# LordLiang/DrawingSpinUp

Hardware: AMD Instinct MI355X
Metric: drawings/sec end-to-end (512x512, 6 views, 24 frames) (higher is better)
Workload: dtype f16 (diffusion) / f16 table + f32 MLP (NSR) / f32 (stage-1 deformable convolutions, IS-Net, contour) / f32 with bf16 x 3 products (stage-2 convolutions; the reference: cuDNN TF32)

## Files before the change

drawingspinup_amd/csrc/hashgrid_mfma.hip:

```cpp
#include "hashgrid_dev.h"
#include "partial_reduce.h"

#include <type_traits>

using namespace dsu_hg;

namespace {

typedef float f32x16 __attribute__((ext_vector_type(16)));
typedef __bf16 bf16x8 __attribute__((ext_vector_type(8)));

__device__ __forceinline__ void softplus_inplace2(f32x16& acc, int r) {
  const f32x2 h = softplus100_pair(f32x2{acc[r], acc[r + 1]});
  acc[r] = h.x;
  acc[r + 1] = h.y;
}

__device__ __forceinline__ void bf16_split8(const float* x, bf16x8& hi, bf16x8& mid) {
#pragma unroll
  for (int i = 0; i < 8; ++i) {
    const __bf16 h = (__bf16)x[i];
    hi[i] = h;
    mid[i] = (__bf16)(x[i] - (float)h);
  }
// ... 922 lines not shown
      for (int l = 0; l < ACT; ++l) vm_take(rw[l]);
      prep_unpack();
      prep_point(e);
      prep_request(e);
      prep_dout(e);
    }
#pragma unroll 1
    for (; e < 7; e += e_step) {
      gb1[0] += dout0;
      const float other0 = partner32(dout0, h);
      const float d0h0 = h == 0 ? dout0 : other0;
      const float d0h1 = h == 1 ? dout0 : other0;
      bf16x8 obh0, obm0, obh1, obm1;
      if constexpr (L0BF)
        pack_operands(in, std::integral_constant<int, (2 * KPA <= 16 ? 2 * KPA : 16)>{}, obh0, obm0, obh1, obm1);
#pragma unroll
      for (int half = 0; half < 2; ++half) {
        if (half == 1 && !live1) break;
        weights_per_use();
        const float d0 = half ? d0h1 : d0h0;
        f32x16 Hh[2];
        if constexpr (L0BF) l0_bf(half ? obh1 : obh0, half ? obm1 : obm0, Hh);
        else l0_half(in, half, Hh);
        softplus2(Hh);
#pragma unroll
        for (int T = 0; T < 2; ++T)
#pragma unroll
          for (int r = 0; r < 16; ++r) gw1c0[T][r] = fmaf(Hh[T][r], d0, gw1c0[T][r]);
        f32x16 din;
#pragma unroll
        for (int r = 0; r < 16; ++r) din[r] = 0.0f;
#pragma unroll
        for (int T = 0; T < 2; ++T) {
          float dpre[16];
#pragma unroll
          for (int q = 0; q < 4; ++q) {
            const float4 w = *reinterpret_cast<const float4*>(&lds[wo + PW_W1O0 + 32 * T + 8 * q + 4 * h]);
            dpre[4 * q + 0] = w.x * d0;
            dpre[4 * q + 1] = w.y * d0;
            dpre[4 * q + 2] = w.z * d0;
            dpre[4 * q + 3] = w.w * d0;
          }
          din_tile(T, dpre, Hh[T], din);
        }
        if (h == half) stage_in_T(in);
        __builtin_amdgcn_wave_barrier();
        gemm_T(gw0, imgI);
        __builtin_amdgcn_wave_barrier();
        store_din(e, din, wave_first + half * 32 + l31, r1);
      }
      const int en = e + e_step < 7 ? e + e_step : 6;
      handover();
      prep_unpack();
      prep_point(en);
      prep_request(en);
      prep_dout(en);
    }
#pragma unroll
    for (int T = 0; T < 2; ++T)
#pragma unroll
      for (int r = 0; r < 16; ++r) {
        float c0 = gw1c0[T][r];
#pragma unroll
        for (int off = 16; off > 0; off >>= 1) c0 += __shfl_xor(c0, off);
        if (l31 == gw1_col(0)) gw0[T][r] += c0;
      }
  }

  __syncthreads();
  float* red = lds;
  {
    float* rr = red + wave * PART_STRIDE;
#pragma unroll
    for (int T = 0; T < 2; ++T)
#pragma unroll
      for (int r = 0; r < 16; ++r) {
        const int feat = feat_of(T, r, h);
        const bool input = l31 < 2 * ACT || (l31 >= 2 * NL && l31 < 2 * NL + 4);
        rr[PART_GW0 + feat * 32 + l31] = input ? gw0[T][r] : 0.0f;
        const int o = l31 >= 2 * NL + 4 ? l31 - (2 * NL + 4) : (l31 >= 2 * ACT && l31 < 2 * ACT + NOUT - 8 ? l31 - 2 * ACT + 8 : -1);
        if (o >= 0) rr[PART_GW1 + feat * 32 + o] = gw0[T][r];
        if (l31 >= NOUT) rr[PART_GW1 + feat * 32 + l31] = 0.0f;
      }
#pragma unroll
    for (int o = 0; o < NOUT; ++o) gb1[o] += __shfl_xor(gb1[o], 32);
#pragma unroll
    for (int off = 16; off > 0; off >>= 1)
#pragma unroll
      for (int o = 0; o < NOUT; ++o) gb1[o] += __shfl_xor(gb1[o], off);
    if (lane == 0) {
#pragma unroll
      for (int o = 0; o < NOUT; ++o) rr[PART_GB1 + o] = gb1[o];
    }
  }
  __syncthreads();
  float* part = partials + (size_t)blockIdx.x * PART_STRIDE;
  for (int v = threadIdx.x; v < PART_GB1 + NOUT; v += blockDim.x)
    part[v] = (red[v] + red[PART_STRIDE + v]) + (red[2 * PART_STRIDE + v] + red[3 * PART_STRIDE + v]);
}

template <int NL, int ACT>
bool launch_bwd_pipe_one(uint32_t active, int blocks, hipStream_t s, const dsu_sdf_mlp& mlp,
                         const float* pts, int64_t n, float radius, float eps, float eps2,
                         const float* d_sdf, const float* d_grad, const float* d_feature,
                         const float* d_laplace, float* partials, const __half2* enc, float2* dinbuf,
                         const int32_t* perm) {
  if ((int)active != ACT) return false;
  sdf_fd_bwd_pipe_kernel<NL, ACT><<<dim3(blocks), dim3(256), 0, s>>>(
      mlp, pts, n, radius, eps, eps2, d_sdf, d_grad, d_feature, d_laplace, partials, enc, dinbuf, perm);
  return true;
}

template <int NL>
bool launch_bwd_pipe(uint32_t active, int blocks, hipStream_t s, const dsu_sdf_mlp& mlp,
                     const float* pts, int64_t n, float radius, float eps, float eps2,
                     const float* d_sdf, const float* d_grad, const float* d_feature,
                     const float* d_laplace, float* partials, const __half2* enc, float2* dinbuf,
                     const int32_t* perm) {
#define DSU_PIPE_TRY(A)                                                                          \
  if (launch_bwd_pipe_one<NL, A>(active, blocks, s, mlp, pts, n, radius, eps, eps2, d_sdf,       \
                                 d_grad, d_feature, d_laplace, partials, enc, dinbuf, perm))      \
    return true;
  DSU_PIPE_TRY(4) DSU_PIPE_TRY(5) DSU_PIPE_TRY(6) DSU_PIPE_TRY(7)
#undef DSU_PIPE_TRY
  return false;
}

constexpr int SC_MAXBLOCKS = 768;
constexpr int SC_THREADS = 256;
constexpr int SC_QCAP = 512;
constexpr int SC_LOG2 = 10;
constexpr int SC_SLOTS = 1 << SC_LOG2;
constexpr int SC_LDS_F = SC_SLOTS + 4 * SC_SLOTS + (SC_THREADS / 64) * 3 * SC_QCAP;
constexpr int SC_TILE_CAP = (SC_LDS_F * 4) / 16;
constexpr int SC_BBOX_OFF = SC_LDS_F;
constexpr int SC_LDS_TOTAL = SC_LDS_F + 16;
static_assert(SC_QCAP % 4 == 0 && SC_QCAP >= 512, "queue: one full evaluation of a wave must fit");

__device__ __forceinline__ uint32_t sc_slot(uint32_t entry) {
  return (entry * 2654435761u) >> (32 - SC_LOG2);
}
__device__ __forceinline__ void sc_commit_from(uint32_t* keys, unsigned long long* acc,
                                               float* __restrict__ gtable, uint32_t entry,
                                               uint32_t slot, float v0, float v1) {
#pragma unroll
  for (int probe = 1; probe < 3; ++probe) {
    slot = (slot + 1) & (SC_SLOTS - 1);
    const uint32_t old = atomicCAS(&keys[slot], GC_EMPTY, entry);
    if (old == GC_EMPTY || old == entry) {
      atomicAdd(&acc[2 * slot], gc_fix(v0));
      atomicAdd(&acc[2 * slot + 1], gc_fix(v1));
      return;
    }
  }
  unsafeAtomicAdd(gtable + (size_t)entry * 2, v0);
  unsafeAtomicAdd(gtable + (size_t)entry * 2 + 1, v1);
}

struct OwnReduce {
  const float* partials;
  int nblocks;
  float *g_w0, *g_b0, *g_w1, *g_b1;
};
constexpr int OWN_RED_BLOCKS = (PART_GB1 + NOUT + 63) / 64;

template <int NL>
__device__ __forceinline__ void reduce_own_block(const OwnReduce& o, int blk, float* red) {
  const int e = threadIdx.x & 63, g = threadIdx.x >> 6, ng = blockDim.x >> 6;
  const int v = blk * 64 + e;
  const bool in_range = v < PART_GB1 + NOUT;
  for (int sl = g; sl < 16; sl += ng) {
    float acc = 0.0f;
    if (in_range)
      for (int b = sl; b < o.nblocks; b += 16) acc += o.partials[(size_t)b * PART_STRIDE + v];
    red[sl * 64 + e] = acc;
  }
  __syncthreads();
  if (g != 0 || !in_range) return;
  float s = 0.0f;
#pragma unroll
  for (int k = 0; k < 16; ++k) s += red[k * 64 + e];
  if (v < PART_GW1) {
    const int feat = v >> 5, k = v & 31;
    if (k < MC<NL>::KIN) {
      const int c = ref_col<NL>(k);
      if (c >= 0) o.g_w0[feat * MC<NL>::DIN + c] += s;
      else o.g_b0[feat] += s;
    }
  } else if (v < PART_GB1) {
    const int feat = (v - PART_GW1) >> 5, oo = (v - PART_GW1) & 31;
    if (oo < NOUT) o.g_w1[oo * HID + feat] += s;
  } else {
    o.g_b1[v - PART_GB1] += s;
  }
}

template <int NL>
__global__ __launch_bounds__(SC_THREADS) void sdf_fd_scatter_kernel(
    GridMeta m, const float* __restrict__ pts, int64_t n, float radius, float eps, uint32_t active,
    const float2* __restrict__ dinbuf, float* __restrict__ gtable, int merge_levels,
    int centre_acc, int dense_levels, int* __restrict__ work_counter, OwnReduce own,
    dsu_partial_reduce extra) {
  extern __shared__ __attribute__((aligned(16))) float lds[];
  const int n_red_own = own.partials ? OWN_RED_BLOCKS : 0;
  const int n_red = n_red_own + (extra.partials ? dsu_red::blocks_of(extra) : 0);
  if ((int)blockIdx.x < n_red) {
    if ((int)blockIdx.x < n_red_own) reduce_own_block<NL>(own, blockIdx.x, lds);
    else dsu_red::reduce_block(extra, blockIdx.x - n_red_own, lds);
    return;
  }
  const int sc_block = (int)blockIdx.x - n_red, sc_grid = (int)gridDim.x - n_red;
  uint32_t* c_keys = reinterpret_cast<uint32_t*>(lds);
  unsigned long long* c_acc = reinterpret_cast<unsigned long long*>(lds + SC_SLOTS);
  const int lane = threadIdx.x & 63, wave = threadIdx.x >> 6;
  float* qbase = lds + 5 * SC_SLOTS + wave * 3 * SC_QCAP;
  uint32_t* q_ent = reinterpret_cast<uint32_t*>(qbase);
  float* q_v0 = qbase + SC_QCAP;
  float* q_v1 = qbase + 2 * SC_QCAP;
  unsigned long long* tile = reinterpret_cast<unsigned long long*>(lds);
  int* bbox = reinterpret_cast<int*>(lds + SC_BBOX_OFF);
  for (int t = threadIdx.x; t < SC_SLOTS; t += blockDim.x) {
    c_keys[t] = GC_EMPTY;
    c_acc[2 * t] = 0ull;
    c_acc[2 * t + 1] = 0ull;
  }
  if (threadIdx.x < 12) bbox[threadIdx.x] = (threadIdx.x % 6) < 3 ? 0x7fffffff : -0x7fffffff;
  int region = 0;
  __syncthreads();
  const int64_t n_chunks = (n + blockDim.x - 1) / blockDim.x;
  const int64_t n_items = n_chunks * (int64_t)active;
  int* next_slot = reinterpret_cast<int*>(lds + SC_BBOX_OFF) + 12;
  int64_t cur = sc_block, nxt = (int64_t)sc_block + sc_grid;
  float pn[3] = {0.f, 0.f, 0.f};
  float2 dnx[7];
#pragma unroll
  for (int e = 0; e < 7; ++e) dnx[e] = make_float2(0.f, 0.f);
  auto request = [&](int64_t item) {
    const int64_t chunk = item / (int64_t)active;
    const uint32_t lv = (uint32_t)(item - chunk * (int64_t)active);
    int64_t idx = chunk * blockDim.x + threadIdx.x;
    idx = idx < n ? idx : n - 1;
    pn[0] = pts[idx * 3]; pn[1] = pts[idx * 3 + 1]; pn[2] = pts[idx * 3 + 2];
#pragma unroll
    for (int e = 0; e < 7; ++e) dnx[e] = dinbuf[((size_t)e * active + lv) * n + idx];
  };
  if (cur < n_items) request(cur);
  int parity = 0;
  int qn = 0;
  auto drain = [&]() {
    __builtin_amdgcn_wave_barrier();
    for (int i0 = 0; i0 < qn; i0 += 64) {
      const int qi = i0 + lane;
      if (qi < qn) {
        const uint32_t ent = q_ent[qi];
        const float a0 = q_v0[qi], a1 = q_v1[qi];
        const uint32_t slot = sc_slot(ent);
        const uint32_t old = atomicCAS(&c_keys[slot], GC_EMPTY, ent);
        if (old == GC_EMPTY || old == ent) {
          atomicAdd(&c_acc[2 * slot], gc_fix(a0));
          atomicAdd(&c_acc[2 * slot + 1], gc_fix(a1));
        } else {
          sc_commit_from(c_keys, c_acc, gtable, ent, slot, a0, a1);
        }
      }
    }
    __builtin_amdgcn_wave_barrier();
    qn = 0;
  };
  auto flush_cache = [&]() {
    for (int t = threadIdx.x; t < SC_SLOTS; t += blockDim.x) {
      const uint32_t key = c_keys[t];
      if (key != GC_EMPTY) {
        unsafeAtomicAdd(gtable + (size_t)key * 2, gc_unfix(c_acc[2 * t]));
        unsafeAtomicAdd(gtable + (size_t)key * 2 + 1, gc_unfix(c_acc[2 * t + 1]));
        c_keys[t] = GC_EMPTY;
        c_acc[2 * t] = 0ull;
        c_acc[2 * t + 1] = 0ull;
      }
    }
  };

#pragma unroll 1
  while (cur < n_items) {
    {
      const int64_t chunk = cur / (int64_t)active;
      const int lev = (int)(cur - chunk * (int64_t)active);
      const float l_scale = m.scale[lev];
      const uint32_t l_off = m.off[lev], hsize = m.off[lev + 1] - m.off[lev];
      const uint32_t l_res = m.res[lev], l_hashed = m.hashed[lev];
      const int64_t i = chunk * blockDim.x + threadIdx.x;
      const bool valid = i < n;
      const float p[3] = {pn[0], pn[1], pn[2]};
      float2 dv[7];
#pragma unroll
      for (int e = 0; e < 7; ++e) {
        dv[e].x = valid ? dnx[e].x : 0.0f;
        dv[e].y = valid ? dnx[e].y : 0.0f;
      }
      if (nxt < n_items) request(nxt);
      if (threadIdx.x == 0) *next_slot = 2 * sc_grid + atomicAdd(work_counter, 1);
      const CellPos ccp = cell_of(l_scale, contract(p[0], radius), contract(p[1], radius),
                                  contract(p[2], radius));
      float2 D0 = dv[0], Da[3];
      uint32_t left = 0u;
      const bool inside = fabsf(p[0]) <= radius && fabsf(p[1]) <= radius && fabsf(p[2]) <= radius;
      int lo[3], hi[3];
#pragma unroll
      for (int a = 0; a < 3; ++a) {
        Da[a] = make_float2(0.f, 0.f);
        lo[a] = valid ? (int)ccp.c[a] : 0x7fffffff;
        hi[a] = valid ? (int)ccp.c[a] : -0x7fffffff;
      }
#pragma unroll
      for (int e = 1; e < 7; ++e) {
        const int ax = (e - 1) >> 1;
        const float off = ((e - 1) & 1) ? -eps : eps;
        const float qa = fminf(fmaxf(p[ax] + off, -radius), radius);
        const float posa = fmaf(l_scale, contract(qa, radius), 0.5f);
        const float fl = floorf(posa);
        const bool same = ((uint32_t)(int)fl == ccp.c[ax]) & (centre_acc != 0) & inside;
        const float delta = posa - ((float)(int)ccp.c[ax] + ccp.f[ax]);
        D0.x += same ? dv[e].x : 0.0f;
        D0.y += same ? dv[e].y : 0.0f;
        Da[ax].x += same ? dv[e].x * delta : 0.0f;
        Da[ax].y += same ? dv[e].y * delta : 0.0f;
        left |= (valid & !same) ? (1u << e) : 0u;
        if (valid & inside) {
          lo[ax] = min(lo[ax], (int)fl);
          hi[ax] = max(hi[ax], (int)fl);
        }
      }
      if (valid & !inside) {
#pragma unroll 1
        for (int e = 1; e < 7; ++e) {
          float q[3];
          fd_point(p, e, eps, radius, q);
          const CellPos cq = cell_of(l_scale, contract(q[0], radius), contract(q[1], radius),
                                     contract(q[2], radius));
#pragma unroll
          for (int a = 0; a < 3; ++a) {
            lo[a] = min(lo[a], (int)cq.c[a]);
            hi[a] = max(hi[a], (int)cq.c[a]);
          }
        }
      }
      bool dense = false;
      int x0 = 0, y0 = 0, z0 = 0, ddx = 1, ddxy = 1, vol = 0;
      int64_t after_next;
      {
        int* bb = bbox + 6 * parity;
#pragma unroll
        for (int a = 0; a < 3; ++a) {
#pragma unroll
          for (int off = 32; off > 0; off >>= 1) {
            lo[a] = min(lo[a], __shfl_xor(lo[a], off));
            hi[a] = max(hi[a], __shfl_xor(hi[a], off));
          }
        }
        if (lane == 0) {
#pragma unroll
          for (int a = 0; a < 3; ++a) {
            atomicMin(&bb[a], lo[a]);
            atomicMax(&bb[3 + a], hi[a]);
          }
        }
        __syncthreads();
        after_next = *next_slot;
        x0 = bb[0]; y0 = bb[1]; z0 = bb[2];
        const long long ex = (long long)bb[3] - x0 + 2, ey = (long long)bb[4] - y0 + 2,
                        ez = (long long)bb[5] - z0 + 2;
        if (dense_levels && bb[3] >= bb[0] && ex * ey * ez <= (long long)SC_TILE_CAP && ex < 4096 && ey < 4096) {
          dense = true;
          ddx = (int)ex; ddxy = (int)(ex * ey); vol = (int)(ex * ey * ez);
        }
        if (threadIdx.x < 6) bbox[6 * (parity ^ 1) + threadIdx.x] = threadIdx.x < 3 ? 0x7fffffff : -0x7fffffff;
        parity ^= 1;
      }
      if ((int)dense != region) {
        if (region == 0) {
          for (int t = threadIdx.x; t < SC_TILE_CAP * 2; t += blockDim.x) tile[t] = 0ull;
        } else {
          for (int t = threadIdx.x; t < SC_SLOTS; t += blockDim.x) {
            c_keys[t] = GC_EMPTY;
            c_acc[2 * t] = 0ull;
            c_acc[2 * t + 1] = 0ull;
          }
        }
        region = (int)dense;
        __syncthreads();
      }

#pragma unroll 1
      for (int e = 1; e < 8; ++e) {
        CellPos cp = ccp;
        float v[16];
        bool flush;
        if (e < 7) {
          flush = (left >> e) & 1u;
          if (__ballot(flush) == 0ull) continue;
          float2 d = dv[1];
#pragma unroll
          for (int k = 2; k < 7; ++k) {
            d.x = e == k ? dv[k].x : d.x;
            d.y = e == k ? dv[k].y : d.y;
          }
          float q[3];
          fd_point(p, e, eps, radius, q);
          cp = cell_of(l_scale, contract(q[0], radius), contract(q[1], radius), contract(q[2], radius));
#pragma unroll
          for (int c = 0; c < 8; ++c) {
            const float w = corner_weight(cp, c);
            v[2 * c] = w * d.x;
            v[2 * c + 1] = w * d.y;
          }
        } else {
          const float X[2] = {1.0f - cp.f[0], cp.f[0]}, Y[2] = {1.0f - cp.f[1], cp.f[1]},
                      Z[2] = {1.0f - cp.f[2], cp.f[2]};
#pragma unroll
          for (int c = 0; c < 8; ++c) {
            const int cx_ = c & 1, cy_ = (c >> 1) & 1, cz_ = (c >> 2) & 1;
            const float yz = Y[cy_] * Z[cz_], xz = X[cx_] * Z[cz_], xy = X[cx_] * Y[cy_];
            const float w = X[cx_] * yz;
            const float gx = cx_ ? yz : -yz, gy = cy_ ? xz : -xz, gz = cz_ ? xy : -xy;
            v[2 * c] = fmaf(D0.x, w, fmaf(Da[0].x, gx, fmaf(Da[1].x, gy, Da[2].x * gz)));
            v[2 * c + 1] = fmaf(D0.y, w, fmaf(Da[0].y, gx, fmaf(Da[1].y, gy, Da[2].y * gz)));
          }
          flush = valid;
        }
        const int key = flush ? (int)((cp.c[0] & 1023u) | ((cp.c[1] & 1023u) << 10) | ((cp.c[2] & 1023u) << 20))
                              : (0x40000000 | lane);
#pragma unroll
        for (int k = 0; k < 16; ++k) v[k] = flush ? v[k] : 0.0f;
        bool lead = flush;
        const int key_next = dpp_i<0x101>(key), key_prev = dpp_i<0x111>(key);
        const int l15 = lane & 15;
        const bool starts = ((l15 == 0) | (key_prev != key)) & flush;
        const int n_flush = __popcll(__ballot(flush)), n_start = __popcll(__ballot(starts));
        if (lev < merge_levels && 4 * n_start <= 3 * n_flush) {
          int ee = ((l15 == 15) | (key_next != key)) ? 1 : 0;
#define DSU_SEG_STEP(CTRL)                                              \
          {                                                             \
            const int eo = dpp_i<CTRL>(ee);                             \
            _Pragma("unroll") for (int k = 0; k < 16; ++k) {            \
              const float vo = dpp_f<CTRL>(v[k]);                       \
              v[k] += ee ? 0.0f : vo;                                   \
            }                                                           \
            ee |= eo;                                                   \
          }
          DSU_SEG_STEP(0x101) DSU_SEG_STEP(0x102) DSU_SEG_STEP(0x104) DSU_SEG_STEP(0x108)
#undef DSU_SEG_STEP
          lead = starts;
        }
        if (dense) {
          if (lead) {
            const int base = ((int)cp.c[0] - x0) + ((int)cp.c[1] - y0) * ddx + ((int)cp.c[2] - z0) * ddxy;
#pragma unroll
            for (int c = 0; c < 8; ++c) {
              const int t = base + (c & 1) + ((c >> 1) & 1) * ddx + ((c >> 2) & 1) * ddxy;
              atomicAdd(&tile[2 * t], gc_fix(v[2 * c]));
              atomicAdd(&tile[2 * t + 1], gc_fix(v[2 * c + 1]));
            }
          }
          continue;
        }
        const unsigned long long bal = __ballot(lead);
        if (lead) {
          const int pos = qn + 8 * __popcll(bal & ((1ull << lane) - 1ull));
          uint32_t ent[8];
#pragma unroll
          for (int c = 0; c < 8; ++c)
            ent[c] = l_off + grid_index(l_hashed, hsize, l_res, cp.c[0] + (c & 1),
                                        cp.c[1] + ((c >> 1) & 1), cp.c[2] + ((c >> 2) & 1));
#pragma unroll
          for (int q4 = 0; q4 < 2; ++q4) {
            *reinterpret_cast<uint4*>(&q_ent[pos + 4 * q4]) =
                make_uint4(ent[4 * q4], ent[4 * q4 + 1], ent[4 * q4 + 2], ent[4 * q4 + 3]);
            *reinterpret_cast<float4*>(&q_v0[pos + 4 * q4]) =
                make_float4(v[8 * q4], v[8 * q4 + 2], v[8 * q4 + 4], v[8 * q4 + 6]);
            *reinterpret_cast<float4*>(&q_v1[pos + 4 * q4]) =
                make_float4(v[8 * q4 + 1], v[8 * q4 + 3], v[8 * q4 + 5], v[8 * q4 + 7]);
          }
        }
        qn += 8 * __popcll(bal);
        if (qn + 512 > SC_QCAP) drain();
      }
      if (!dense) drain();
      __syncthreads();
      if (dense) {
        for (int t = threadIdx.x; t < vol; t += blockDim.x) {
          const unsigned long long a0 = tile[2 * t], a1 = tile[2 * t + 1];
          if (a0 | a1) {
            const int z = t / ddxy, rr = t - z * ddxy;
            const int y = rr / ddx, x = rr - y * ddx;
            const uint32_t g = l_off + grid_index(l_hashed, hsize, l_res, (uint32_t)(x0 + x),
                                                  (uint32_t)(y0 + y), (uint32_t)(z0 + z));
            unsafeAtomicAdd(gtable + (size_t)g * 2, gc_unfix(a0));
            unsafeAtomicAdd(gtable + (size_t)g * 2 + 1, gc_unfix(a1));
            tile[2 * t] = 0ull;
            tile[2 * t + 1] = 0ull;
          }
        }
      } else {
        flush_cache();
      }
      cur = nxt;
      nxt = after_next;
    }
  }
}

constexpr int BWD_MFMA_MAX_BLOCKS = 512;

}

#define DSU_DISPATCH_NL(nl, ...)                       \
  switch (nl) {                                        \
    case 10: { constexpr int NL = 10; __VA_ARGS__ } break; \
    case 12: { constexpr int NL = 12; __VA_ARGS__ } break; \
    default: return DSU_EUNSUP;                        \
  }

extern "C" {

int64_t dsu_sdf_fd_enc_cache_bytes(int64_t n, uint32_t active_levels) {
  if (n < 0 || active_levels > DSU_MAX_LEVELS) return DSU_EINVAL;
  return (int64_t)7 * n * active_levels * 4;
}

int64_t dsu_sdf_fd_bwd_workspace_bytes(const dsu_hashgrid_cfg* cfg, int64_t n) {
  if (!cfg || n < 0) return DSU_EINVAL;
  if (cfg->n_levels != 10 && cfg->n_levels != 12) return DSU_EUNSUP;
  const int blocks = dsu_capped_blocks(n, 256, BWD_MFMA_MAX_BLOCKS);
  return (int64_t)blocks * PART_STRIDE * sizeof(float) +
         (int64_t)7 * n * cfg->n_levels * (int64_t)sizeof(float2) + 256;
}

int dsu_sdf_fd_bwd_sorted(const dsu_hashgrid_cfg* cfg, const void* table_f16, const dsu_sdf_mlp* mlp,
                   const float* pts, const int32_t* perm, int64_t n, float radius, float eps,
                   uint32_t active_levels, const float* d_sdf, const float* d_grad,
                   const float* d_feature, const float* d_laplace, float* grad_table,
                   float* g_w0, float* g_b0, float* g_w1, float* g_b1, void* workspace,
                   int64_t workspace_bytes, const void* enc_cache, void* stream) {
  return dsu_sdf_fd_bwd_sorted_mid(cfg, table_f16, mlp, pts, perm, n, radius, eps, active_levels,
                                   d_sdf, d_grad, d_feature, d_laplace, grad_table, g_w0, g_b0, g_w1,
                                   g_b1, workspace, workspace_bytes, enc_cache, nullptr, stream);
}

int dsu_sdf_fd_bwd_sorted_mid(const dsu_hashgrid_cfg* cfg, const void* table_f16,
                              const dsu_sdf_mlp* mlp, const float* pts, const int32_t* perm,
                              int64_t n, float radius, float eps, uint32_t active_levels,
                              const float* d_sdf, const float* d_grad, const float* d_feature,
                              const float* d_laplace, float* grad_table, float* g_w0, float* g_b0,
                              float* g_w1, float* g_b1, void* workspace, int64_t workspace_bytes,
                              const void* enc_cache, void* mid_event, void* stream) {
  return dsu_sdf_fd_bwd_sorted_fold(cfg, table_f16, mlp, pts, perm, n, radius, eps, active_levels,
                                    d_sdf, d_grad, d_feature, d_laplace, grad_table, g_w0, g_b0, g_w1,
                                    g_b1, workspace, workspace_bytes, enc_cache, mid_event, nullptr,
                                    stream);
}

int dsu_sdf_fd_bwd_sorted_fold(const dsu_hashgrid_cfg* cfg, const void* table_f16,
                               const dsu_sdf_mlp* mlp, const float* pts, const int32_t* perm,
                               int64_t n, float radius, float eps, uint32_t active_levels,
                               const float* d_sdf, const float* d_grad, const float* d_feature,
                               const float* d_laplace, float* grad_table, float* g_w0, float* g_b0,
                               float* g_w1, float* g_b1, void* workspace, int64_t workspace_bytes,
                               const void* enc_cache, void* mid_event,
                               const dsu_partial_reduce* extra, void* stream) {
  if (extra && (!extra->partials || !extra->map || !extra->base || extra->nblocks < 0 ||
                extra->n <= 0 || extra->stride < extra->n))
    return DSU_EINVAL;
  if (extra && n == 0) return DSU_EUNSUP;
  if (!cfg || !table_f16 || !mlp || (!pts && n) || n < 0) return DSU_EINVAL;
  if (!mlp->w0 || !mlp->b0 || !mlp->w1 || !mlp->b1) return DSU_EINVAL;
  if (!grad_table || !g_w0 || !g_b0 || !g_w1 || !g_b1) return DSU_EINVAL;
  if (active_levels > cfg->n_levels || !(eps > 0.0f)) return DSU_EINVAL;
  GridMeta m;
  int rc = make_meta(cfg, &m);
  if (rc) return rc;
  for (uint32_t l = 0; l < active_levels; ++l)
    if (m.res[l] + 1u > 1024u) return DSU_EUNSUP;
  if (n == 0) return DSU_OK;
  const int64_t need = dsu_sdf_fd_bwd_workspace_bytes(cfg, n);
  if (need < 0) return (int)need;
  if (!workspace || workspace_bytes < need) return DSU_EINVAL;
  hipStream_t s = (hipStream_t)stream;
  const float eps2 = (float)((double)eps * (double)eps);
  const int blocks = dsu_onewave_blocks(n, 256, BWD_MFMA_MAX_BLOCKS);
  const size_t shm1 = (size_t)K1_LDS_F * sizeof(float);
  const size_t shm2 = (size_t)SC_LDS_TOTAL * sizeof(float);
  float2* dinbuf = reinterpret_cast<float2*>((char*)workspace +
                                             (size_t)blocks * PART_STRIDE * sizeof(float));
  int sblocks = dsu_capped_blocks(n, SC_THREADS, SC_MAXBLOCKS);
  if (dsu_scatter_grid_cap_value > 0 && sblocks > dsu_scatter_grid_cap_value) sblocks = dsu_scatter_grid_cap_value;
  DSU_DISPATCH_NL(cfg->n_levels, {
    auto k1 = enc_cache ? sdf_fd_bwd_mfma_kernel<NL, true> : sdf_fd_bwd_mfma_kernel<NL, false>;
    auto k2 = sdf_fd_scatter_kernel<NL>;
    DSU_ENSURE_DYN_LDS((sdf_fd_bwd_mfma_kernel<NL, true>), shm1);
    DSU_ENSURE_DYN_LDS((sdf_fd_bwd_mfma_kernel<NL, false>), shm1);
    DSU_ENSURE_DYN_LDS(k2, shm2);
    bool piped = false;
    if constexpr (NL == 10) {
      if (enc_cache)
        piped = launch_bwd_pipe<NL>(active_levels, blocks, s, *mlp, pts, n, radius, eps, eps2,
                                    d_sdf, d_grad, d_feature, d_laplace, (float*)workspace,
                                    (const __half2*)enc_cache, dinbuf, perm);
    }
    if (!piped)
      k1<<<dim3(blocks), dim3(256), shm1, s>>>(
          (const __half2*)table_f16, m, *mlp, pts, n, radius, eps, eps2, active_levels, d_sdf,
          d_grad, d_feature, d_laplace, (float*)workspace, (const __half2*)enc_cache, dinbuf, perm);
    if (mid_event && hipEventRecord((hipEvent_t)mid_event, s) != hipSuccess) return DSU_ELAUNCH;
    int* work_counter = reinterpret_cast<int*>(dinbuf + (size_t)7 * (size_t)n * cfg->n_levels);
    const OwnReduce own{(const float*)workspace, blocks, g_w0, g_b0, g_w1, g_b1};
    dsu_partial_reduce ext{};
    if (extra) ext = *extra;
    const int n_red = OWN_RED_BLOCKS + (extra ? dsu_red::blocks_of(ext) : 0);
    k2<<<dim3(n_red + sblocks), dim3(SC_THREADS), shm2, s>>>(m, pts, n, radius, eps, active_levels,
                                                            dinbuf, grad_table,  64,
                                                             1,  1,
                                                            work_counter, own, ext);
  });
  DSU_CHECK_LAUNCH();
  return DSU_OK;
}

int dsu_sdf_fd_bwd_cached(const dsu_hashgrid_cfg* cfg, const void* table_f16,
                          const dsu_sdf_mlp* mlp, const float* pts, int64_t n, float radius,
                          float eps, uint32_t active_levels, const float* d_sdf,
                          const float* d_grad, const float* d_feature, const float* d_laplace,
                          float* grad_table, float* g_w0, float* g_b0, float* g_w1, float* g_b1,
                          void* workspace, int64_t workspace_bytes, const void* enc_cache,
                          void* stream) {
  return dsu_sdf_fd_bwd_sorted(cfg, table_f16, mlp, pts, nullptr, n, radius, eps, active_levels,
                               d_sdf, d_grad, d_feature, d_laplace, grad_table, g_w0, g_b0, g_w1,
                               g_b1, workspace, workspace_bytes, enc_cache, stream);
}

int dsu_sdf_fd_bwd(const dsu_hashgrid_cfg* cfg, const void* table_f16, const dsu_sdf_mlp* mlp,
                   const float* pts, int64_t n, float radius, float eps,
                   uint32_t active_levels, const float* d_sdf, const float* d_grad,
                   const float* d_feature, const float* d_laplace, float* grad_table,
                   float* g_w0, float* g_b0, float* g_w1, float* g_b1, void* workspace,
                   int64_t workspace_bytes, void* stream) {
  return dsu_sdf_fd_bwd_sorted(cfg, table_f16, mlp, pts, nullptr, n, radius, eps, active_levels,
                               d_sdf, d_grad, d_feature, d_laplace, grad_table, g_w0, g_b0, g_w1,
                               g_b1, workspace, workspace_bytes, nullptr, stream);
}

}
```

Before: 0.3437.

## Fold adjacent-cell finite-difference scatters into centre and face passes

Finite-difference sample points that fall into the cell next to the centre cell are no longer scattered as full 8-corner trilinear updates. The four corners they share with the centre cell are folded into the centre pass, and the far face gets a dedicated per-axis 4-corner pass carrying a hit mask through the segmented DPP reduction. This cuts the number of full scatter iterations and atomics or queue entries for points near the centre cell. In exchange the loop has more iterations, more register state (fa, adj, hb) and more complex index arithmetic, and some atomics in the dense path are skipped via the mask.

```diff
diff --git a/drawingspinup_amd/csrc/hashgrid_mfma.hip b/drawingspinup_amd/csrc/hashgrid_mfma.hip
--- a/drawingspinup_amd/csrc/hashgrid_mfma.hip
+++ b/drawingspinup_amd/csrc/hashgrid_mfma.hip
@@ -1248,7 +1248,9 @@
       const CellPos ccp = cell_of(l_scale, contract(p[0], radius), contract(p[1], radius),
                                   contract(p[2], radius));
       float2 D0 = dv[0], Da[3];
-      uint32_t left = 0u;
+      uint32_t left = 0u, adj = 0u;
+      float fa[7];
+      fa[0] = 0.0f;
       const bool inside = fabsf(p[0]) <= radius && fabsf(p[1]) <= radius && fabsf(p[2]) <= radius;
       int lo[3], hi[3];
 #pragma unroll
@@ -1270,7 +1272,11 @@
         D0.y += same ? dv[e].y : 0.0f;
         Da[ax].x += same ? dv[e].x * delta : 0.0f;
         Da[ax].y += same ? dv[e].y * delta : 0.0f;
-        left |= (valid & !same) ? (1u << e) : 0u;
+        const int rel = (int)fl - (int)ccp.c[ax];
+        const bool adjacent = (rel == (((e - 1) & 1) ? -1 : 1)) & (centre_acc != 0) & inside;
+        fa[e] = posa - fl;
+        left |= (valid & !same & !adjacent) ? (1u << e) : 0u;
+        adj |= (valid & adjacent) ? (1u << e) : 0u;
         if (valid & inside) {
           lo[ax] = min(lo[ax], (int)fl);
           hi[ax] = max(hi[ax], (int)fl);
@@ -1337,10 +1343,13 @@
       }
 
 #pragma unroll 1
-      for (int e = 1; e < 8; ++e) {
+      for (int e = 1; e < 11; ++e) {
         CellPos cp = ccp;
         float v[16];
         bool flush;
+        int hb = 3;
+        const int A = (e >= 7 && e < 10) ? e - 7 : 2;
+        const int p_lo = (e >= 7 && e < 10) ? -1 : 0, p_hi = (e >= 7 && e < 10) ? 2 : 1;
         if (e < 7) {
           flush = (left >> e) & 1u;
           if (__ballot(flush) == 0ull) continue;
@@ -1359,17 +1368,56 @@
             v[2 * c] = w * d.x;
             v[2 * c + 1] = w * d.y;
           }
+        } else if (e < 10) {
+          const bool ap = (adj >> (2 * A + 1)) & 1u, am = (adj >> (2 * A + 2)) & 1u;
+          flush = ap | am;
+          if (__ballot(flush) == 0ull) continue;
+          float2 dp = dv[1], dm = dv[2];
+          float fp = fa[1], fm = fa[2];
+#pragma unroll
+          for (int k = 1; k < 3; ++k) {
+            dp.x = A == k ? dv[2 * k + 1].x : dp.x;
+            dp.y = A == k ? dv[2 * k + 1].y : dp.y;
+            dm.x = A == k ? dv[2 * k + 2].x : dm.x;
+            dm.y = A == k ? dv[2 * k + 2].y : dm.y;
+            fp = A == k ? fa[2 * k + 1] : fp;
+            fm = A == k ? fa[2 * k + 2] : fm;
+          }
+          const float f1 = A == 0 ? ccp.f[1] : ccp.f[0], f2 = A == 2 ? ccp.f[1] : ccp.f[2];
+          const float wl = am ? 1.0f - fm : 0.0f, wh = ap ? fp : 0.0f;
+          const float2 Glo = make_float2(dm.x * wl, dm.y * wl), Ghi = make_float2(dp.x * wh, dp.y * wh);
+          const float B1[2] = {1.0f - f1, f1}, B2[2] = {1.0f - f2, f2};
+#pragma unroll
+          for (int j = 0; j < 4; ++j) {
+            const float o = B1[j & 1] * B2[j >> 1];
+            v[2 * j] = Glo.x * o;
+            v[2 * j + 1] = Glo.y * o;
+            v[8 + 2 * j] = Ghi.x * o;
+            v[8 + 2 * j + 1] = Ghi.y * o;
+          }
+          hb = (am ? 1 : 0) | (ap ? 2 : 0);
         } else {
           const float X[2] = {1.0f - cp.f[0], cp.f[0]}, Y[2] = {1.0f - cp.f[1], cp.f[1]},
                       Z[2] = {1.0f - cp.f[2], cp.f[2]};
+          float2 Fn[3], Ff[3];
+#pragma unroll
+          for (int a = 0; a < 3; ++a) {
+            const float wn = ((adj >> (2 * a + 2)) & 1u) ? fa[2 * a + 2] : 0.0f;
+            const float wf = ((adj >> (2 * a + 1)) & 1u) ? 1.0f - fa[2 * a + 1] : 0.0f;
+            Fn[a] = make_float2(dv[2 * a + 2].x * wn, dv[2 * a + 2].y * wn);
+            Ff[a] = make_float2(dv[2 * a + 1].x * wf, dv[2 * a + 1].y * wf);
+          }
 #pragma unroll
           for (int c = 0; c < 8; ++c) {
             const int cx_ = c & 1, cy_ = (c >> 1) & 1, cz_ = (c >> 2) & 1;
             const float yz = Y[cy_] * Z[cz_], xz = X[cx_] * Z[cz_], xy = X[cx_] * Y[cy_];
             const float w = X[cx_] * yz;
             const float gx = cx_ ? yz : -yz, gy = cy_ ? xz : -xz, gz = cz_ ? xy : -xy;
-            v[2 * c] = fmaf(D0.x, w, fmaf(Da[0].x, gx, fmaf(Da[1].x, gy, Da[2].x * gz)));
-            v[2 * c + 1] = fmaf(D0.y, w, fmaf(Da[0].y, gx, fmaf(Da[1].y, gy, Da[2].y * gz)));
+            const float2 fx = cx_ ? Ff[0] : Fn[0], fy = cy_ ? Ff[1] : Fn[1], fz = cz_ ? Ff[2] : Fn[2];
+            const float s0 = fmaf(D0.x, w, fmaf(Da[0].x, gx, fmaf(Da[1].x, gy, Da[2].x * gz)));
+            const float s1 = fmaf(D0.y, w, fmaf(Da[0].y, gx, fmaf(Da[1].y, gy, Da[2].y * gz)));
+            v[2 * c] = fmaf(fx.x, yz, fmaf(fy.x, xz, fmaf(fz.x, xy, s0)));
+            v[2 * c + 1] = fmaf(fx.y, yz, fmaf(fy.y, xz, fmaf(fz.y, xy, s1)));
           }
           flush = valid;
         }
@@ -1377,6 +1425,7 @@
                               : (0x40000000 | lane);
 #pragma unroll
         for (int k = 0; k < 16; ++k) v[k] = flush ? v[k] : 0.0f;
+        hb = flush ? hb : 0;
         bool lead = flush;
         const int key_next = dpp_i<0x101>(key), key_prev = dpp_i<0x111>(key);
         const int l15 = lane & 15;
@@ -1387,10 +1436,12 @@
 #define DSU_SEG_STEP(CTRL)                                              \
           {                                                             \
             const int eo = dpp_i<CTRL>(ee);                             \
+            const int ho = dpp_i<CTRL>(hb);                             \
             _Pragma("unroll") for (int k = 0; k < 16; ++k) {            \
               const float vo = dpp_f<CTRL>(v[k]);                       \
               v[k] += ee ? 0.0f : vo;                                   \
             }                                                           \
+            hb |= ee ? 0 : ho;                                          \
             ee |= eo;                                                   \
           }
           DSU_SEG_STEP(0x101) DSU_SEG_STEP(0x102) DSU_SEG_STEP(0x104) DSU_SEG_STEP(0x108)
@@ -1398,13 +1449,19 @@
           lead = starts;
         }
         if (dense) {
-          if (lead) {
-            const int base = ((int)cp.c[0] - x0) + ((int)cp.c[1] - y0) * ddx + ((int)cp.c[2] - z0) * ddxy;
-#pragma unroll
-            for (int c = 0; c < 8; ++c) {
-              const int t = base + (c & 1) + ((c >> 1) & 1) * ddx + ((c >> 2) & 1) * ddxy;
-              atomicAdd(&tile[2 * t], gc_fix(v[2 * c]));
-              atomicAdd(&tile[2 * t + 1], gc_fix(v[2 * c + 1]));
+          const int sA = A == 0 ? 1 : A == 1 ? ddx : ddxy;
+          const int s1 = A == 0 ? ddx : 1, s2 = A == 2 ? ddx : ddxy;
+          const int base = ((int)cp.c[0] - x0) + ((int)cp.c[1] - y0) * ddx + ((int)cp.c[2] - z0) * ddxy;
+#pragma unroll
+          for (int h = 0; h < 2; ++h) {
+            if (lead && ((hb >> h) & 1)) {
+#pragma unroll
+              for (int j = 0; j < 4; ++j) {
+                const int c = 4 * h + j;
+                const int t = base + (j & 1) * s1 + (j >> 1) * s2 + (h ? p_hi : p_lo) * sA;
+                atomicAdd(&tile[2 * t], gc_fix(v[2 * c]));
+                atomicAdd(&tile[2 * t + 1], gc_fix(v[2 * c + 1]));
+              }
             }
           }
           continue;
@@ -1414,9 +1471,12 @@
           const int pos = qn + 8 * __popcll(bal & ((1ull << lane) - 1ull));
           uint32_t ent[8];
 #pragma unroll
-          for (int c = 0; c < 8; ++c)
-            ent[c] = l_off + grid_index(l_hashed, hsize, l_res, cp.c[0] + (c & 1),
-                                        cp.c[1] + ((c >> 1) & 1), cp.c[2] + ((c >> 2) & 1));
+          for (int c = 0; c < 8; ++c) {
+            const int pl = (c >> 2) ? p_hi : p_lo, b1 = c & 1, b2 = (c >> 1) & 1;
+            const int dx = A == 0 ? pl : b1, dy = A == 1 ? pl : A == 0 ? b1 : b2, dz = A == 2 ? pl : b2;
+            ent[c] = l_off + grid_index(l_hashed, hsize, l_res, cp.c[0] + (uint32_t)dx,
+                                        cp.c[1] + (uint32_t)dy, cp.c[2] + (uint32_t)dz);
+          }
 #pragma unroll
           for (int q4 = 0; q4 < 2; ++q4) {
             *reinterpret_cast<uint4*>(&q_ent[pos + 4 * q4]) =
```

Measured after the change: 0.3402. 0.99x the previous value.
